# kongan/PL-SLAM-plucker

Measured on AMD Instinct MI355X. Metric: LM iterations/sec (and ms/iter) on local-BA window; final χ² vs g2o, higher is better.
Workload: dtype f64; 1 GPU; C3: 100 KF (10 fixed) / 20000 points / 4000 Plücker lines, 93975+18441 edges; one independent window per GPU; edges=112416, survey_nominal_edges=120000, trials_per_lba=23, factorisation=two-sided column-lane band LDLT (bw 7), parallelism=1 independent windows (1 per GPU)

## Files before the change

### pl-slam-plucker_amd/csrc/plba.hip

```cpp
#include <hip/hip_runtime.h>
#include <rccl/rccl.h>

#include <algorithm>
#include <chrono>
#include <cmath>
#include <cstdarg>
#include <cstdio>
#include <cstring>
#include <limits>
#include <map>
#include <mutex>
#include <numeric>
#include <string>
#include <type_traits>
#include <utility>
#include <vector>

#include "../../include/plba.h"
#include "plba_build.hpp"
#include "plba_kernels.hpp"
#include "plba_plan.hpp"
#include "plba_scratch.hpp"

namespace plba {
// ... 944 lines not shown
        d.bcr_sl[1] = N * (int64_t)bcr_xrec(bw);
        d.bcr_sl[2] = N * (int64_t)bcr_X_doubles(bw);
        d.bcr_sl[3] = 2 * N;
        d.bcr_sl[4] = kBcrCtl;
        d.bcr_sl[5] = N * (int64_t)kBcrStamps;
        ALLOC(d.bcr_pub, (size_t)W * d.bcr_sl[0]);
        ALLOC(d.bcr_x, (size_t)W * d.bcr_sl[1]);
        ALLOC(d.bcr_X, (size_t)W * d.bcr_sl[2]);
        h.h_kf.assign(nf, 0);
        for (int k = 0; k < n_kf; ++k)
            if (ws.kf_hidx[k] >= 0) h.h_kf[ws.kf_hidx[k]] = k;
        UPLOAD(d.h_kf, h.h_kf);
        ZALLOC(d.bcr_flag, (size_t)W * d.bcr_sl[3]);
        ZALLOC(d.bcr_ctl, (size_t)W * kBcrCtl);
        ZALLOC(d.bcr_stamps, (size_t)W * d.bcr_sl[5]);
        ALLOC(ctx->bk_T, (size_t)n_kf * 12);
        ALLOC(ctx->bk_X, (size_t)std::max(n_lm, 1) * 4);
        ALLOC(ctx->bk_xp, (size_t)std::max(n, 6));
        ALLOC(ctx->bk_xk, (size_t)n_kf * 6);
        ALLOC(ctx->bk_Lpb, (size_t)std::max(n_ln, 1) * 8);
        ALLOC(ctx->bk_XL, (size_t)std::max(n_ln_g, 1) * 6);
        ALLOC(ctx->bk_level, (size_t)std::max(E, 1));
        ALLOC(ctx->bk_xl, (size_t)std::max(n_lm, 1) * 4);
    }
    if (!d.band_mode) ZALLOC(d.bcr_stamps, kBcrStamps);
    ALLOC(d.bs, (size_t)W * n);
    for (int b = 0; b < nbx; ++b) ZALLOC(d.xpb[b], std::max(n, 6));
    ALLOC(d.Wbuf, (size_t)std::max(n, 1) * (kTile + 1));
    UPLOAD(d.tile_first, bp.tile_first);
    UPLOAD(d.tile_last, bp.tile_last);
    ALLOC(d.part_chi2, d.n_lin_blocks);
    ALLOC(d.part_any, d.n_lm_blocks);
    ALLOC(d.part_max, nf + d.n_lm_blocks);
    ALLOC(d.pose_part, (size_t)std::max(nf, 1) * kPoseParts * kPP);
    ALLOC(d.part_lm, (size_t)W * sl_lms(d));
    ALLOC(d.part_lms, (size_t)W * sl_lms(d));
    const int nred = kPoseParts * nf + (d.n_lm > 0 ? d.n_lm_blocks : 0), ngrp = (nred + kRedGrp - 1) / kRedGrp;
    ZALLOC(d.cnt, 2 + (size_t)nblk + nf + ngrp);
    ZALLOC(d.cnt_rcs, (size_t)W * nblk);
    ALLOC(d.wg_red, 3 * (size_t)std::max(nred, 1));
    ALLOC(d.grp_red, 3 * (size_t)std::max(ngrp, 1));
    d.n_ps = std::max(d.n_kf_blocks, d.bcr_N);
    ZALLOC(d.part_ps, (size_t)W * d.n_ps);
    ZALLOC(d.ctrl, 1);
    ALLOC(d.trace, kTraceCap);
    ALLOC(ctx->d_depth, Ep);
    ALLOC(d.red_rcs, (size_t)nblk * 36 + (size_t)nf * 6);
    ALLOC(d.red_dec, 3);
    if (d.sharded) {
        ALLOC(d.red_rcs_loc, (size_t)nblk * 36 + (size_t)nf * 6);
        ALLOC(d.red_dec_loc, 4);
    }
    d.xg_P = 0;
    if (d.sharded && xg.rng.size()) {
        d.xg_P = xg.P;
        UPLOAD(d.xg_rng, xg.rng);
        ZALLOC(d.xg_send, (size_t)(d.xg_host ? R : 1) * xg.P);
        ALLOC(d.xg_recv, (size_t)R * xg.P);
    }
    UPLOAD_D(d.lm_gpos, ctx->lm_gpos, wb.lm_gpos, n_lm);
    UPLOAD_D(d.e_gpos, ws.e_gpos, wb.e_gpos, E);
    if (d.sharded) {
        ALLOC(d.gat, (size_t)d.n_lm_g * 4 + 3 * (size_t)d.E_g);
    } else {
        ALLOC(ctx->d_outd, out_doubles(n_kf, n_pt, n_ln, E) + ((size_t)Ep + E + 7) / 8);
    }
#if defined(PLBA_STAMPS) || defined(PLBA_PHASE_STAMPS) || defined(PLBA_LMS_STAMPS)
    ZALLOC(d.stamps, 17 * 8);
#endif
}
#undef ALLOC
#undef ZALLOC
#undef UPLOAD
#undef UPLOAD_D
int stage_arrays(plba_ctx *ctx, const plba_graph *g, const WindowStructure &ws, const BlockPattern &bp,
                 const ShardRanges &xg, PhaseLog &mark) {
    StagedHost h;
    stage_state_arrays(ctx, g, ws, h);
    stage_system_arrays(ctx, g, ws, bp, xg, h);
    mark("host arrays staged");
    return ctx->commit_plan();
}
void bind_views(Dev &d) {
    const size_t nf = (size_t)d.nf;
    d.xp = d.xpb[0];
    d.xl = d.xlb[0];
    d.chi2_last = d.chi2b[0];
    if (d.sharded) {
        d.Hpp = nullptr;
        d.Hdg = d.red_iter;
        d.bp = d.red_iter + nf * 6;
        d.pact = d.red_iter + nf * 12;
        d.Hdg_w = d.red_iter_loc;
        d.bp_w = d.red_iter_loc + nf * 6;
        d.pact_w = d.red_iter_loc + nf * 12;
    } else {
        d.Hpp = d.red_iter;
        d.bp = d.red_iter + nf * 36;
        d.pact = d.red_iter + nf * 42;
        d.red_iter_loc = d.red_iter;
// ... 79 lines not shown
        return PLBA_OK;
    }
    ctx->set_error("sharded window without a transport");
    return PLBA_E_COMM;
}
int allgather(plba_ctx *ctx, const double *send, double *recv, size_t P) {
    auto &c = ctx->comm;
    if (P == 0) return PLBA_OK;
    if (c.kind == plba_ctx::Comm::RCCL) {
        const ncclResult_t r = ncclAllGather(send, recv, P, ncclDouble, c.nccl, ctx->stream);
        if (r != ncclSuccess) {
            ctx->set_error("ncclAllGather(%zu doubles): %s", P, ncclGetErrorString(r));
            return PLBA_E_COMM;
        }
        return PLBA_OK;
    }
    return allreduce(ctx, send, recv, (size_t)c.nranks * P);
}
#define COMM(send, recv, n)                                                        \
    do {                                                                           \
        int _crc = 0;                                                              \
        LAUNCH(K_COMM, _crc = allreduce(ctx, (send), (recv), (size_t)(n)));        \
        if (_crc) return _crc;                                                     \
    } while (0)

bool chunk_half(const plba_ctx *ctx) { return (long long)ctx->d.nch > ctx->tuning.chunk_half_min; }
int launch_step(plba_ctx *ctx) {
    Dev &d = ctx->d;
    hipStream_t s = ctx->stream;
    const bool chunk_direct = ctx->tuning.chunk_direct;

    if (d.E > 0) LAUNCH(K_LINEARIZE, hipLaunchKernelGGL(k_linearize, dim3(d.n_lin_blocks), dim3(kBlock), 0, s, d));
    if (d.nf > 0 || d.n_lm > 0) {
        const int nred = kPoseParts * d.nf + (d.n_lm > 0 ? d.n_lm_blocks : 0);
        LAUNCH(K_REDUCE, hipLaunchKernelGGL(k_iter_reduce, dim3(nred), dim3(kLmBlock), 0, s, d));
    }
    if (d.sharded) {
        LAUNCH(K_PACK, hipLaunchKernelGGL(k_iter_pack, dim3(1), dim3(kInitNT), 0, s, d));
        COMM(d.red_iter_loc, d.red_iter, (size_t)d.nf * 13 + 2 + d.nranks);
    }
    const bool reduced = d.nf > 0 || d.n_lm > 0;
    if (!(d.fold_init && reduced))
        LAUNCH(K_ITER_INIT, hipLaunchKernelGGL(k_iter_init, dim3(1), dim3(kInitNT), 0, s, d));
    if (d.n_lm > 0) {
        LAUNCH(K_ESCHUR, hipLaunchKernelGGL(k_edge_schur, dim3(d.n_lin_blocks, d.spec_max), dim3(kBlock), 0, s, d));
    }
    if (d.n > 0) {
        if (!d.band_mode) LAUNCH(K_MEMSET, (void)hipMemsetAsync(d.Ad, 0, sizeof(double) * (size_t)d.n * d.n, s));
        if (d.nch > 0) LAUNCH(K_ASSEMBLE, hipLaunchKernelGGL(chunk_direct ? k_rcs_chunk<false> : chunk_half(ctx) ? k_rcs_chunk_h : k_rcs_chunk<true>, dim3(8 * ((d.nch + 7) / 8), d.spec_max), dim3(64), 0, s, d));
        if (d.sharded) {
            LAUNCH(K_PACK, hipLaunchKernelGGL(k_rcs_blockpart, dim3(blocks_for(d.nblk * 42)), dim3(kBlock), 0, s, d));
            if (d.xg_P > 0) {
                int grc = 0;
                LAUNCH(K_COMM, grc = allgather(ctx, d.xg_send, d.xg_recv, (size_t)d.xg_P));
                if (grc) return grc;
                LAUNCH(K_FINALIZE, hipLaunchKernelGGL(k_rcs_xunpack, dim3(blocks_for(d.nblk * 36 + d.nf * 6)), dim3(kBlock), 0, s, d));
            } else {
                COMM(d.red_rcs_loc, d.red_rcs, (size_t)d.nblk * 36 + (size_t)d.nf * 6);
            }
        }
        if (!(d.fold && d.nch > 0))
            LAUNCH(K_FINALIZE, hipLaunchKernelGGL(k_rcs_finalize, dim3(blocks_for(d.nblk * 42)), dim3(kBlock), 0, s, d));
        const size_t solve_lds = d.n <= d.solve_lds_n ? sizeof(double) * (size_t)d.n : 0;
        if (d.band_mode) {
            hipError_t fe = hipSuccess;
            LAUNCH(K_FACTOR, fe = launch_band(d, s));
            if (fe != hipSuccess) {
                (void)hipGetLastError();
// ... 779 lines not shown
        PLBA_CHECK(d2h(ctx, res->kf_x, d.xk[ctx->cur], sizeof(double) * (size_t)d.n_kf * 6));
    }
    if (gba && res->ln_line3d && ctx->n_ln)
        PLBA_CHECK(d2h(ctx, res->ln_line3d, d.XL[ctx->cur], sizeof(double) * (size_t)ctx->n_ln * 6));
    return plba_download(ctx, res->kf_Tcw, res->pt_xyz, gba ? nullptr : res->ln_orth);
}

int plba_get_trace(plba_ctx *ctx, plba_iter_trace *out, int32_t cap, int32_t *n) {
    if (!ctx) return PLBA_E_INVALID;
    if (n) *n = (int32_t)ctx->trace.size();
    if (out)
        for (int i = 0; i < (int)ctx->trace.size() && i < cap; ++i) out[i] = ctx->trace[i];
    return PLBA_OK;
}

int plba_synchronize(plba_ctx *ctx) {
    if (!ctx) return PLBA_E_INVALID;
    PLBA_CHECK(hipStreamSynchronize(ctx->stream));
    return PLBA_OK;
}

int plba_kernel_times(plba_ctx *ctx, const char **names, double *ms, int32_t *launches, int32_t cap, int32_t *n) {
    if (!ctx) return PLBA_E_INVALID;
    if (n) *n = K_COUNT;
    for (int k = 0; k < K_COUNT && k < cap; ++k) {
        if (names) names[k] = kKernelNames[k];
        if (ms) ms[k] = ctx->k_ms[k];
        if (launches) launches[k] = ctx->k_n[k];
    }
    return PLBA_OK;
}

int plba_debug_stamps(plba_ctx *ctx, unsigned long long *out ) {
#if defined(PLBA_STAMPS) || defined(PLBA_PHASE_STAMPS) || defined(PLBA_LMS_STAMPS)
    if (!ctx || !ctx->d.stamps) return PLBA_E_STATE;
    PLBA_CHECK(d2h(ctx, out, ctx->d.stamps, 17 * 8 * sizeof(unsigned long long)));
    return PLBA_OK;
#else
    (void)ctx; (void)out;
    return PLBA_E_STATE;
#endif
}

int plba_debug_bcr_stamps(plba_ctx *ctx, unsigned long long *out, int32_t cap, int32_t *rows) {
    if (!ctx || !out || !rows) return PLBA_E_INVALID;
    if (!ctx->uploaded || !ctx->d.bcr_stamps) return PLBA_E_STATE;
    const int rows_ = std::max(ctx->d.bcr_N, 1);
    const int n = std::min(cap / kBcrStamps, rows_);
    *rows = rows_;
    PLBA_CHECK(d2h(ctx, out, ctx->d.bcr_stamps, sizeof(unsigned long long) * (size_t)n * kBcrStamps));
    return PLBA_OK;
}

int plba_structure_stats(plba_ctx *ctx, int64_t *out, int32_t cap) {
    if (!ctx || !out) return PLBA_E_INVALID;
    if (!ctx->uploaded) return PLBA_E_STATE;
    const int64_t v[22] = {ctx->d.nf, ctx->d.bw, ctx->d.nblk, (int64_t)ctx->n_triples, ctx->d.E, ctx->d.n_lm,
                           ctx->d.band_mode, ctx->d.nch, ctx->n_free_edges, ctx->d.Ep,
                           ctx->step_exec != nullptr, ctx->d.sharded, ctx->d.twisted, ctx->d.cl, ctx->d.bcr_N,
                           ctx->d.dense_mfma, ctx->bcr_fallbacks, ctx->d.spec_max, ctx->d.spec_policy,
                           ctx->h_ctrl ? ctx->h_ctrl->steps : 0, ctx->d.bcr_fused, ctx->dev_build};
    for (int i = 0; i < cap && i < 22; ++i) out[i] = v[i];
    return PLBA_OK;
}

int plba_factor_plan(int32_t bw, int32_t nf, int32_t resident, int32_t flags, int32_t *out, int32_t cap) {
    if (!out || bw < 0 || nf < 0) return PLBA_E_INVALID;
// ... 208 lines not shown
```

### pl-slam-plucker_amd/csrc/plba_dev.hpp

```cpp
#pragma once

#include <hip/hip_runtime.h>
#include <stdint.h>

#include "../../include/plba.h"
#include "plba_math.hpp"

namespace plba {

constexpr int kBlock = 256;
constexpr int kLmBlock = 64;
constexpr int kChunk = 256;
constexpr int kTraceCap = 64;
constexpr int kTile = 32;
constexpr int kBandMax = 27;
constexpr int kBandNT = 768;
__host__ __device__ constexpr int band_nt(int bw) { return bw <= 24 ? kBandNT : 512; }
__host__ __device__ constexpr int band_ur(int bw) { return band_nt(bw) <= 512 ? 6 : 3; }
constexpr int kMaxSpec = 4;
constexpr int kNB = kMaxSpec + 1;

enum LmKind : int32_t {
    kLmG2o = 0,
    kLmLbaPlucker = 1,
// ... 75 lines not shown
    int32_t bw, band_mode;
    int32_t dense_mfma;
    int32_t ring;
    unsigned long long *stamps;
    int32_t *first_blk;
    double *Bd;
    double *Lband;
    double *Kinv;
    double *zb;
    double *part_chi2;
    double *wg_red, *grp_red;
    int32_t *part_any;
    double *part_max;
    double *part_lm, *part_lms;
    double *part_ps;
    int32_t n_ps;
    int32_t fold;
    int32_t fold_init;
    int32_t *cnt;
    int32_t *h_kf;
    Ctrl *ctrl;
    plba_iter_trace *trace;
    int32_t sharded, nranks, rank;
    int32_t n_lm_g, E_g;
    double *red_iter, *red_iter_loc;
    double *red_rcs, *red_rcs_loc;
    double *xg_send, *xg_recv;
    int64_t *xg_rng;
    int64_t xg_P;
    int32_t xg_host;
    double *red_dec, *red_dec_loc;
    double *Hpp_w, *bp_w;
    double *Hdg, *Hdg_w;
    double *pose_part;
    double *pact, *pact_w;
    int32_t *lm_gpos, *e_gpos;
    double *gat;
    int32_t cl;
    int32_t diag;
    int32_t twisted, tw_m;
    double *Bd2, *bs2;
    double *Lband2, *Kinv2, *zb2;
    double *tw_sep;
    int32_t *tw_fail, *tw_count;
    int32_t bcr, bcr_N;
    int32_t bcr_fused;
    double *bcr_pub;
    double *bcr_x;
    double *bcr_X;
    uint32_t *bcr_flag;
    uint32_t *bcr_ctl;
    unsigned long long *bcr_stamps;
    int64_t bcr_sl[6];
};


__device__ __forceinline__ double *Tcur(const Dev &d) { return d.Tb[d.ctrl->cur]; }
__device__ __forceinline__ double *Xcur(const Dev &d) { return d.Xb[d.ctrl->cur]; }
__device__ __forceinline__ double *chi2cur(const Dev &d) { return d.chi2b[d.ctrl->chi_src]; }

__host__ __device__ __forceinline__ size_t sl_band(const Dev &d) { return d.band_mode ? (size_t)d.nf * (d.bw + 1) * 36 : 1; }
__host__ __device__ __forceinline__ size_t sl_tw(const Dev &d) { return (size_t)d.nf * (d.bw + 1) * 36; }
__host__ __device__ __forceinline__ size_t sl_sep(const Dev &d) {
    return 2 * ((size_t)d.bw * (d.bw + 1) * 36 + (size_t)d.bw * 6);
}
__host__ __device__ __forceinline__ size_t sl_chp(const Dev &d) { return (size_t)(d.nch > 1 ? d.nch : 1) * 42; }
__host__ __device__ __forceinline__ size_t sl_lms(const Dev &d) { return (size_t)(d.n_lms_blocks > 1 ? d.n_lms_blocks : 1); }
// ... 156 lines not shown
```

### pl-slam-plucker_amd/csrc/plba_kernels.hpp

```cpp
#pragma once

#include "plba_dev.hpp"

namespace plba {

__global__ __launch_bounds__(kBlock) void k_linearize(Dev d) {
    ITER_GUARD
    __shared__ double sh[kBlock / 64];
    const int e = blockIdx.x * kBlock + threadIdx.x;
    double rc = 0.0;
    const Ctrl *cc = d.ctrl;
    const bool sw = cc->switch_pending;
    const int nxt = cc->stage + 1;
    const int robust = sw ? cc->stage_robust[nxt] : cc->robust;
    double *chi2e = chi2cur(d);
    __shared__ __attribute__((aligned(16))) double stA[kBlock * 12], stc[kBlock * 2], stB[kBlock * 8];
    if (e < d.E) {
        double *A = stA + threadIdx.x * 12, *c = stc + threadIdx.x * 2, *B = stB + threadIdx.x * 8;
        if (sw) {
            const double stale = chi2e[e];
            for (int b = 0; b < d.nbx; ++b)
                if (d.chi2b[b] != chi2e) d.chi2b[b][e] = stale;
            if (cc->stage_classify[nxt]) {
                bool bad = stale > kChi2Thr;
// ... 80 lines not shown
            const double s = sqrt(rho1 * info);
            const bool pose_free = d.e_hidx[e] >= 0;
#pragma unroll
            for (int k = 0; k < 12; ++k) A[k] = pose_free ? s * Jp[k] : 0.0;
            c[0] = -s * err[0];
            c[1] = -s * err[1];
#pragma unroll
            for (int k = 0; k < 8; ++k) B[k] = s * Jl[k];
        } else {
#pragma unroll
            for (int k = 0; k < 12; ++k) A[k] = 0.0;
            c[0] = c[1] = 0.0;
#pragma unroll
            for (int k = 0; k < 8; ++k) B[k] = 0.0;
        }
    }
    __syncthreads();
    {
        const int e0 = blockIdx.x * kBlock, n = min(kBlock, d.E - e0);
        auto copy_out = [&](const double *src, double *dst, int cnt) {
            const double2 *s2 = reinterpret_cast<const double2 *>(src);
            double2 *d2 = reinterpret_cast<double2 *>(dst);
            for (int t = threadIdx.x; t < cnt / 2; t += kBlock) d2[t] = s2[t];
        };
        copy_out(stA, d.A + (size_t)e0 * 12, n * 12);
        copy_out(stc, d.cvec + (size_t)e0 * 2, n * 2);
        copy_out(stB, d.B + (size_t)e0 * 8, n * 8);
    }
    double s = block_sum<kBlock>(rc, sh);
    if (threadIdx.x == 0) d.part_chi2[blockIdx.x] = s;
}

constexpr int kPoseParts = 4;
constexpr int kPoseKU = 4;
constexpr int kPP = 28;
constexpr int kInitNT = 1024;

__device__ __forceinline__ constexpr int pk(int r, int c) { return r * (r + 1) / 2 + c; }

__device__ __forceinline__ double pose_partial(const Dev &d, int h, int part) {
    double acc[kPP];
#pragma unroll
    for (int k = 0; k < kPP; ++k) acc[k] = 0.0;
    constexpr int S = kPoseParts * 64, kU = kPoseKU;
    const int pend = d.pe_off[h + 1];
    for (int p0 = d.pe_off[h] + part * 64 + threadIdx.x; p0 < pend; p0 += kU * S) {
        int ei[kU];
#pragma unroll
        for (int j = 0; j < kU; ++j) ei[j] = p0 + j * S < pend ? d.pe_list[p0 + j * S] : -1;
        double a[kU][12], cv[kU][2];
#pragma unroll
        for (int j = 0; j < kU; ++j) {
            const int e = ei[j] < 0 ? ei[0] : ei[j];
            const double *A = d.A + (size_t)e * 12;
#pragma unroll
            for (int k = 0; k < 12; ++k) a[j][k] = A[k];
            cv[j][0] = d.cvec[(size_t)e * 2];
            cv[j][1] = d.cvec[(size_t)e * 2 + 1];
        }
#pragma unroll
        for (int j = 0; j < kU; ++j) {
            if (ei[j] < 0) break;
            acc[27] += d.e_active[ei[j]] ? 1.0 : 0.0;
            const double *a0 = a[j], *a1 = a[j] + 6;
            int idx = 0;
#pragma unroll
            for (int r = 0; r < 6; ++r)
#pragma unroll
                for (int cc = r; cc < 6; ++cc) acc[idx++] += a0[r] * a0[cc] + a1[r] * a1[cc];
#pragma unroll
            for (int r = 0; r < 6; ++r) acc[21 + r] += a0[r] * cv[j][0] + a1[r] * cv[j][1];
        }
    }
    {
        const int lane = threadIdx.x;
        double v[32];
#pragma unroll
        for (int k = 0; k < 32; ++k) v[k] = k < kPP ? acc[k] : 0.0;
#pragma unroll
        for (int n = 16; n >= 1; n >>= 1) {
            const int m = 2 * n;
            const bool hi = (lane & m) != 0;
#pragma unroll
            for (int i = 0; i < n; ++i) {
                const double keep = hi ? v[n + i] : v[i], send = hi ? v[i] : v[n + i];
                v[i] = keep + __shfl_xor(send, m, 64);
            }
        }
        v[0] += __shfl_xor(v[0], 1, 64);
        if ((lane & 1) == 0 && lane / 2 < kPP)
            st_sc1(d.pose_part + ((size_t)h * kPoseParts + part) * kPP + lane / 2, v[0]);
    }
    if ((d.fold_init || d.sharded) && arrive_last(d.cnt + 2 + d.nblk + h, kPoseParts)) {
        const int k = threadIdx.x;
        double v = 0.0;
        if (k < kPP) {
            const double *src = d.pose_part + (size_t)h * kPoseParts * kPP + k;
            double p[kPoseParts];
#pragma unroll
            for (int j = 0; j < kPoseParts; ++j) p[j] = ld_sc1(src + j * kPP);
            v = p[0];
#pragma unroll
            for (int j = 1; j < kPoseParts; ++j) v += p[j];
            if (k < 21) {
                int r = 0, rem = k;
                while (rem >= 6 - r) { rem -= 6 - r; ++r; }
                const int cc = r + rem;
                d.Hpp_w[(size_t)h * 36 + r * 6 + cc] = v;
                d.Hpp_w[(size_t)h * 36 + cc * 6 + r] = v;
                if (r == cc && d.Hdg_w) d.Hdg_w[(size_t)h * 6 + r] = v;
                if (r != cc) v = 0.0;
            } else if (k < 27) {
                d.bp_w[(size_t)h * 6 + (k - 21)] = v;
                v = 0.0;
            } else {
                d.pact_w[h] = v;
                v = 0.0;
            }
        }
        const double m = wave_max(fabs(v));
        if (threadIdx.x == 0) st_sc1(d.part_max + h, m);
        return m;
    }
    return 0.0;
}

__device__ __forceinline__ void landmark_reduce(const Dev &d, int lb, double &mx_out, int &any_out) {
    __shared__ double sh[kLmBlock / 64];
    const int l = lb * kLmBlock + threadIdx.x;
    const bool sw = d.ctrl->switch_pending;
    double mx = 0.0;
    bool any = false;
    if (l < d.n_lm) {
        if (sw) {
            bool act = false;
            for (int e = d.lm_off[l]; e < d.lm_off[l + 1]; ++e) act = act || d.e_active[e];
            d.lm_active[l] = act ? 1 : 0;
        }
        any = d.lm_active[l] != 0;
        if (l >= d.n_pt && lm_endpoint_lines(d.ctrl->hlm)) {
            double H6[21], b6[6];
#pragma unroll
            for (int k = 0; k < 21; ++k) H6[k] = 0.0;
#pragma unroll
            for (int k = 0; k < 6; ++k) b6[k] = 0.0;
            for (int e = d.lm_off[l]; e < d.lm_off[l + 1]; ++e) {
                double bb[6];
#pragma unroll
                for (int k = 0; k < 6; ++k) bb[k] = d.B[(size_t)e * 8 + k];
                const double c0 = d.cvec[(size_t)e * 2];
#pragma unroll
                for (int r = 0; r < 6; ++r) {
#pragma unroll
                    for (int cc = 0; cc <= r; ++cc) H6[pk(r, cc)] += bb[r] * bb[cc];
                    b6[r] += bb[r] * c0;
                }
            }
            const int li = l - d.n_pt;
#pragma unroll
            for (int k = 0; k < 21; ++k) d.Hl6[(size_t)li * 21 + k] = H6[k];
#pragma unroll
            for (int k = 0; k < 6; ++k) d.bl6[(size_t)li * 6 + k] = b6[k];
// ... 5 lines not shown
        for (int k = 0; k < 10; ++k) H[k] = 0.0;
#pragma unroll
        for (int k = 0; k < 4; ++k) b[k] = 0.0;
        const int e1 = d.lm_off[l + 1];
        for (int e0 = d.lm_off[l]; e0 < e1; e0 += 2) {
            double bb[2][8], cc2[2][2];
#pragma unroll
            for (int j = 0; j < 2; ++j) {
                const int e = e0 + j < e1 ? e0 + j : e0;
#pragma unroll
                for (int k = 0; k < 8; ++k) bb[j][k] = d.B[(size_t)e * 8 + k];
                cc2[j][0] = d.cvec[(size_t)e * 2];
                cc2[j][1] = d.cvec[(size_t)e * 2 + 1];
            }
#pragma unroll
            for (int j = 0; j < 2; ++j) {
                if (e0 + j >= e1) break;
                const double *b0 = bb[j], *b1 = bb[j] + 4;
#pragma unroll
                for (int r = 0; r < 4; ++r) {
#pragma unroll
                    for (int cc = 0; cc <= r; ++cc) H[pk(r, cc)] += b0[r] * b0[cc] + b1[r] * b1[cc];
                    b[r] += b0[r] * cc2[j][0] + b1[r] * cc2[j][1];
                }
            }
        }
#pragma unroll
        for (int k = 0; k < 10; ++k) d.Hll[(size_t)l * 10 + k] = H[k];
#pragma unroll
        for (int k = 0; k < 4; ++k) d.bl[(size_t)l * 4 + k] = b[k];
        mx = fmax(fmax(fabs(H[pk(0, 0)]), fabs(H[pk(1, 1)])), fmax(fabs(H[pk(2, 2)]), fabs(H[pk(3, 3)])));
        }
    }
    double m = block_max<kLmBlock>(mx, sh);
    const int anyb = __syncthreads_or(any ? 1 : 0);
    if (threadIdx.x == 0) {
        st_sc1(d.part_max + d.nf + lb, m);
        __hip_atomic_store(d.part_any + lb, anyb, __ATOMIC_RELAXED, __HIP_MEMORY_SCOPE_AGENT);
    }
    mx_out = m;
    any_out = anyb;
}


template <int NT, bool SC1 = false>
__device__ __forceinline__ double pose_combine(const Dev &d, double *H, double *bp) {
    double m = 0.0;
    for (int i = threadIdx.x; i < d.nf * kPP; i += NT) {
        const int h = i / kPP, k = i % kPP;
        const double *src = d.pose_part + (size_t)h * kPoseParts * kPP + k;
        double v = SC1 ? ld_sc1(src) : src[0];
#pragma unroll
        for (int j = 1; j < kPoseParts; ++j) v += SC1 ? ld_sc1(src + j * kPP) : src[j * kPP];
        if (k < 21) {
            int r = 0, rem = k;
            while (rem >= 6 - r) { rem -= 6 - r; ++r; }
            const int cc = r + rem;
            H[(size_t)h * 36 + r * 6 + cc] = v;
            H[(size_t)h * 36 + cc * 6 + r] = v;
            if (r == cc) m = fmax(m, fabs(v));
        } else if (k < 27) {
            bp[(size_t)h * 6 + (k - 21)] = v;
        } else {
            d.pact_w[h] = v;
        }
    }
    return m;
}

__global__ __launch_bounds__(kInitNT) void k_iter_pack(Dev d) {
    ITER_GUARD
    __shared__ double sh[kInitNT / 64];
    double s = 0.0;
    for (int i = threadIdx.x; i < d.n_lin_blocks; i += kInitNT) s += d.part_chi2[i];
    const double chi = block_sum<kInitNT>(s, sh);
    double m = 0.0;
    for (int i = threadIdx.x; i < d.n_lm_blocks; i += kInitNT) m = fmax(m, d.part_max[d.nf + i]);
    const double mx = block_max<kInitNT>(m, sh);
    int any = 0;
    for (int i = threadIdx.x; i < d.n_lm_blocks; i += kInitNT) any |= d.part_any[i];
    any = __syncthreads_or(any);
    double *o = d.red_iter_loc + (size_t)d.nf * 13;
    if (threadIdx.x == 0) {
        o[0] = chi;
        o[1] = any ? 1.0 : 0.0;
    }
    for (int r = threadIdx.x; r < d.nranks; r += kInitNT) o[2 + r] = r == d.rank ? mx : 0.0;
}

__device__ __forceinline__ void iter_init_ctrl(const Dev &d, double chi, double mx, bool any);
template <int NT>
__device__ __forceinline__ void iter_init_body(const Dev &d, double *sh) {
    double chi, mx;
    bool any;
    if (d.sharded) {
        const double *o = d.red_iter + (size_t)d.nf * 13;
        double m = 0.0;
        for (int i = threadIdx.x; i < d.nf * 6; i += NT) m = fmax(m, fabs(d.Hdg[i]));
        for (int r = threadIdx.x; r < d.nranks; r += NT) m = fmax(m, o[2 + r]);
        mx = block_max<NT>(m, sh);
        chi = o[0];
        any = o[1] != 0.0;
    } else {
        double m = pose_combine<NT>(d, d.Hpp_w, d.bp_w);
        double s = 0.0;
        for (int i = threadIdx.x; i < d.n_lin_blocks; i += NT) s += d.part_chi2[i];
        chi = block_sum<NT>(s, sh);
        for (int i = threadIdx.x; i < d.n_lm_blocks; i += NT) m = fmax(m, d.part_max[d.nf + i]);
        mx = block_max<NT>(m, sh);
        int a = 0;
        for (int i = threadIdx.x; i < d.n_lm_blocks; i += NT) a |= d.part_any[i];
        any = __syncthreads_or(a) != 0;
    }
    if (threadIdx.x == 0) iter_init_ctrl(d, chi, mx, any);
}
__device__ __forceinline__ void iter_init_ctrl(const Dev &d, double chi, double mx, bool any) {
    {
        Ctrl *c = d.ctrl;
        if (c->switch_pending) {
            c->switch_pending = 0;
            c->stage += 1;
            c->iter = 0;
            c->robust = c->stage_robust[c->stage];
            c->level = c->stage_level[c->stage];
            if (!any) {
                c->iters_done[c->stage] = -1;
                c->chi2_final[c->stage] = 0.0;
                c->need_iter = 0;
                if (c->stage + 1 < c->n_stages) c->switch_pending = 1;
                else c->all_done = 1;
                return;
            }
        }
        if (lm_hand_rolled(c->hlm)) {
            const double err = chi / (c->hlm == kLmLbaEndpoints && c->iter > 0 ? c->hlm_nobs2 : c->hlm_nobs);
            c->hlm_lin += 1;
            if (c->iter == 0) {
                c->maxdiag = mx;
                c->lambda = c->hlm_lambda0 * (c->hlm == kLmGba ? (double)(long long)mx : mx);
            } else if (fabs(err - c->err_prev) < c->hlm_minchg || err < c->hlm_minerr) {
                if (c->ntrace < kTraceCap)
// ... 2 lines not shown
                c->chi2_final[c->stage] = err;
                c->need_iter = 0;
                c->all_done = 1;
                return;
            }
            c->currentChi = err;
            c->chi2_start = err;
            c->lambda_start = c->lambda;
            c->accept = 0;
            c->need_iter = 0;
            return;
        }
        if (c->iter == 0) {
            c->currentChi = chi;
            c->maxdiag = mx;
            c->lambda = d.tau * mx;
            c->ni = 2.0;
        }
        c->chi2_start = c->currentChi;
        c->lambda_start = c->lambda;
        c->qmax = 0;
        c->accept = 0;
        c->rho = 0.0;
        c->broke = 0;
        c->need_iter = 0;
    }
}
__global__ __launch_bounds__(kInitNT) void k_iter_init(Dev d) {
    ITER_GUARD
    __shared__ double sh[kInitNT / 64];
    iter_init_body<kInitNT>(d, sh);
}

constexpr int kRedGrp = 256;
__device__ __forceinline__ bool iter_init_fast(const Dev &d) {
    const Ctrl *c = d.ctrl;
    return d.fold_init && !d.sharded && !lm_hand_rolled(c->hlm) && !c->switch_pending && c->iter > 0;
}
__global__ __launch_bounds__(kLmBlock) void k_iter_reduce(Dev d) {
    ITER_GUARD
    __shared__ double sh_init[kLmBlock / 64];
    const int b = blockIdx.x, np = kPoseParts * d.nf;
    const int G = (int)gridDim.x, lane = threadIdx.x;
    double sc = 0.0;
    if (d.fold_init && !iter_init_fast(d)) {
        const int lo = (int)((long long)b * d.n_lin_blocks / G), hi = (int)((long long)(b + 1) * d.n_lin_blocks / G);
        for (int i = lo + lane; i < hi; i += kLmBlock) sc += d.part_chi2[i];
    }
    double wmax = 0.0;
    int wany = 0;
    if (b < np) wmax = pose_partial(d, b / kPoseParts, b % kPoseParts);
    else landmark_reduce(d, b - np, wmax, wany);
    if (!d.fold_init) return;
    if (iter_init_fast(d)) return;
    {
        sc = wave_sum(sc);
        if (lane == 0) {
            st_sc1(d.wg_red + 3 * (size_t)b, sc);
            st_sc1(d.wg_red + 3 * (size_t)b + 1, wmax);
            st_sc1(d.wg_red + 3 * (size_t)b + 2, wany ? 1.0 : 0.0);
        }
    }
    constexpr int U = kRedGrp / kLmBlock;
    const int g = b / kRedGrp, gn = min(kRedGrp, G - kRedGrp * g), ng = (G + kRedGrp - 1) / kRedGrp;
    if (!arrive_last(d.cnt + 2 + d.nblk + d.nf + g, gn)) return;
    {
        double cv[U], mv[U], av[U];
#pragma unroll
        for (int u = 0; u < U; ++u) {
            const int k = lane * U + u;
            const double *w = d.wg_red + 3 * (size_t)(kRedGrp * g + min(k, gn - 1));
            cv[u] = ld_sc1(w);
            mv[u] = ld_sc1(w + 1);
            av[u] = ld_sc1(w + 2);
        }
        double c = 0.0, m = 0.0, a = 0.0;
#pragma unroll
        for (int u = 0; u < U; ++u)
            if (lane * U + u < gn) {
                c += cv[u];
                m = fmax(m, mv[u]);
                a = fmax(a, av[u]);
            }
        c = wave_sum(c);
        m = wave_max(m);
        a = wave_max(a);
        if (lane == 0) {
            st_sc1(d.grp_red + 3 * (size_t)g, c);
            st_sc1(d.grp_red + 3 * (size_t)g + 1, m);
            st_sc1(d.grp_red + 3 * (size_t)g + 2, a);
        }
    }
    if (!arrive_last(d.cnt + 1, ng)) return;
    double c = 0.0, m = 0.0, a = 0.0;
    for (int g0 = 0; g0 < ng; g0 += 64) {
        double cg = 0.0, mg = 0.0, ag = 0.0;
        if (g0 + lane < ng) {
            const double *w = d.grp_red + 3 * (size_t)(g0 + lane);
            cg = ld_sc1(w);
            mg = ld_sc1(w + 1);
            ag = ld_sc1(w + 2);
        }
        c += wave_sum(cg);
        m = fmax(m, wave_max(mg));
        a = fmax(a, wave_max(ag));
    }
    (void)sh_init;
    if (lane == 0) iter_init_ctrl(d, c, m, a != 0.0);
}

}

#include "plba_rcs.hpp"
#include "plba_dense.hpp"
#include "plba_band.hpp"
#include "plba_band_cl.hpp"
#include "plba_bcr.hpp"
#include "plba_pgo.hpp"

namespace plba {

__global__ __launch_bounds__(kBlock) void k_pose_update(Dev d0) {
    TRIAL_SLOT(0)
    if (blockIdx.x == 0) pose_update_wg<kBlock>(d, false);
}

__device__ __forceinline__ void lm_chol(const Dev &d, int l, double lam, bool mul, double (&L)[10], double (&g)[4],
                                        double (&S)[4], bool sgn = false) {
    const int DIM = is_point_lm(d, l) ? 3 : 4;
    double H[10];
#pragma unroll
    for (int k = 0; k < 10; ++k) { H[k] = d.Hll[(size_t)l * 10 + k]; L[k] = 0.0; }
#pragma unroll
    for (int k = 0; k < 4; ++k) { g[k] = 0.0; S[k] = 1.0; }
#pragma unroll
    for (int j = 0; j < 4; ++j) {
        if (j < DIM) {
            double sj = H[pk(j, j)] + (mul ? lam * H[pk(j, j)] : lam);
#pragma unroll
            for (int p = 0; p < j; ++p) sj -= (L[pk(j, p)] * S[p]) * L[pk(j, p)];
// ... 796 lines not shown
```

### pl-slam-plucker_amd/plba/roofline.py

```python
from __future__ import annotations

from .synth import Graph

F = 8
I = 4


def state_bytes(g: Graph) -> int:
    return g.n_kf * 12 * F + g.n_pt * 3 * F + g.n_ln * 4 * F


def kernel_bytes(g: Graph, name: str, st: dict) -> float:
    E, Ep, El = g.n_ept + g.n_eln, g.n_ept, g.n_eln
    Ef = st.get("free_edges", E)
    n_lm = g.n_pt + g.n_ln
    nf = st.get("nf", int((g.kf_fixed == 0).sum()))
    bw = st.get("bw", 7)
    T = st.get("triples", 0)
    nblk = st.get("nblk", 0)
    nch = st.get("chunks", 0)
    blk = 36 * F
    if name == "k_linearize":
        rd = Ep * (2 * I + 2 * F + F + 1 + I) + El * (2 * I + 4 * F + F + 1 + I) + state_bytes(g)
        return rd + E * (12 + 2 + 8 + 1) * F
    if name == "k_iter_reduce":
        return (Ef * (I + 14 * F) + nf * 4 * 27 * F
                + E * (8 + 2) * F + n_lm * (I + (10 + 4) * F))
    if name == "k_iter_init":
        return nf * 4 * 27 * F + nf * (36 + 6) * F
    if name == "k_edge_schur":
        return E * (I + 8 * F + 10 * F) + n_lm * (10 + 4) * F
    if name == "k_rcs_chunk":
        return E * (12 + 8 + 2) * F + T * 2 * I + nch * 42 * F
    if name == "k_rcs_finalize":
        return nch * 42 * F + nf * (36 + 6) * F + nblk * blk + nf * 6 * F
    if name in ("k_rcs_factor", "k_rcs_factor_band", "k_rcs_factor_twisted"):
        return (nf * (bw + 1) * blk + nf * 6 * F + nf * bw * blk + nf * (36 + 6 + 6) * F
                + g.n_kf * (12 + 12) * F + nf * 6 * F)
    if name == "k_rcs_factor_bcr":
        S = 6 * bw
        N = -(-nf // max(bw, 1))
        NG = (2 * bw + 1) * (2 * bw + 2) // 2 - 1
        return (nf * (bw + 1) * blk + nf * 6 * F + (N - 1) * 36 * NG * F * 3 + N * S * F * 3
                + nf * 6 * F + g.n_kf * (12 + 12) * F + nf * 6 * F)
    if name == "k_pose_update":
        return g.n_kf * (12 + 12) * F + nf * 12 * F
    if name == "k_lm_solve":
        ev = Ep * (I + 1 + 2 * F + F) + El * (I + 1 + 4 * F + F) + E * F + g.n_kf * 12 * F
        return n_lm * (4 + 4 + 10 + 4 + 4) * F + n_lm * I + Ef * (I + (12 + 8) * F) + nf * 6 * F + ev
    return 0.0
```

Baseline: 5478 LM iterations/s.

## Fuse per-pose partial reductions into one workgroup via LDS instead of global atomics

k_iter_reduce now runs one 256-thread workgroup per free pose, with four waves, in place of four separate 64-thread workgroups. The four pose partials are combined in shared memory behind a barrier. Before, they went through global pose_part storage plus an arrive-last atomic counter, and pose_combine ran again in iter_init. Landmark blocks are packed four waves per workgroup, and the grouped final reduction uses groups of 64. The aim is to cut the workgroup count, global round-trips and atomic synchronisation in the per-iteration reduction. Optional cycle-counter instrumentation (PLBA_IRP_STAMPS) is also added.

```diff
diff --git a/pl-slam-plucker_amd/csrc/plba.hip b/pl-slam-plucker_amd/csrc/plba.hip
--- a/pl-slam-plucker_amd/csrc/plba.hip
+++ b/pl-slam-plucker_amd/csrc/plba.hip
@@ -1000,11 +1000,10 @@
     ALLOC(d.part_chi2, d.n_lin_blocks);
     ALLOC(d.part_any, d.n_lm_blocks);
     ALLOC(d.part_max, nf + d.n_lm_blocks);
-    ALLOC(d.pose_part, (size_t)std::max(nf, 1) * kPoseParts * kPP);
     ALLOC(d.part_lm, (size_t)W * sl_lms(d));
     ALLOC(d.part_lms, (size_t)W * sl_lms(d));
-    const int nred = kPoseParts * nf + (d.n_lm > 0 ? d.n_lm_blocks : 0), ngrp = (nred + kRedGrp - 1) / kRedGrp;
-    ZALLOC(d.cnt, 2 + (size_t)nblk + nf + ngrp);
+    const int nred = iter_reduce_wgs(d), ngrp = (nred + kRedGrp - 1) / kRedGrp;
+    ZALLOC(d.cnt, 2 + (size_t)ngrp);
     ZALLOC(d.cnt_rcs, (size_t)W * nblk);
     ALLOC(d.wg_red, 3 * (size_t)std::max(nred, 1));
     ALLOC(d.grp_red, 3 * (size_t)std::max(ngrp, 1));
@@ -1033,7 +1032,9 @@
     } else {
         ALLOC(ctx->d_outd, out_doubles(n_kf, n_pt, n_ln, E) + ((size_t)Ep + E + 7) / 8);
     }
-#if defined(PLBA_STAMPS) || defined(PLBA_PHASE_STAMPS) || defined(PLBA_LMS_STAMPS)
+#if defined(PLBA_IRP_STAMPS) && PLBA_IRP_STAMPS == 2
+    ZALLOC(d.stamps, 17 * 8 + (size_t)nf * (1 + kPoseParts * kPP));
+#elif defined(PLBA_STAMPS) || defined(PLBA_PHASE_STAMPS) || defined(PLBA_LMS_STAMPS) || defined(PLBA_IRP_STAMPS)
     ZALLOC(d.stamps, 17 * 8);
 #endif
 }
@@ -1179,8 +1180,7 @@
 
     if (d.E > 0) LAUNCH(K_LINEARIZE, hipLaunchKernelGGL(k_linearize, dim3(d.n_lin_blocks), dim3(kBlock), 0, s, d));
     if (d.nf > 0 || d.n_lm > 0) {
-        const int nred = kPoseParts * d.nf + (d.n_lm > 0 ? d.n_lm_blocks : 0);
-        LAUNCH(K_REDUCE, hipLaunchKernelGGL(k_iter_reduce, dim3(nred), dim3(kLmBlock), 0, s, d));
+        LAUNCH(K_REDUCE, hipLaunchKernelGGL(k_iter_reduce, dim3(iter_reduce_wgs(d)), dim3(kRedNT), 0, s, d));
     }
     if (d.sharded) {
         LAUNCH(K_PACK, hipLaunchKernelGGL(k_iter_pack, dim3(1), dim3(kInitNT), 0, s, d));
@@ -2026,7 +2026,7 @@
 }
 
 int plba_debug_stamps(plba_ctx *ctx, unsigned long long *out ) {
-#if defined(PLBA_STAMPS) || defined(PLBA_PHASE_STAMPS) || defined(PLBA_LMS_STAMPS)
+#if defined(PLBA_STAMPS) || defined(PLBA_PHASE_STAMPS) || defined(PLBA_LMS_STAMPS) || defined(PLBA_IRP_STAMPS)
     if (!ctx || !ctx->d.stamps) return PLBA_E_STATE;
     PLBA_CHECK(d2h(ctx, out, ctx->d.stamps, 17 * 8 * sizeof(unsigned long long)));
     return PLBA_OK;
diff --git a/pl-slam-plucker_amd/csrc/plba_dev.hpp b/pl-slam-plucker_amd/csrc/plba_dev.hpp
--- a/pl-slam-plucker_amd/csrc/plba_dev.hpp
+++ b/pl-slam-plucker_amd/csrc/plba_dev.hpp
@@ -131,7 +131,6 @@
     double *red_dec, *red_dec_loc;
     double *Hpp_w, *bp_w;
     double *Hdg, *Hdg_w;
-    double *pose_part;
     double *pact, *pact_w;
     int32_t *lm_gpos, *e_gpos;
     double *gat;
diff --git a/pl-slam-plucker_amd/csrc/plba_kernels.hpp b/pl-slam-plucker_amd/csrc/plba_kernels.hpp
--- a/pl-slam-plucker_amd/csrc/plba_kernels.hpp
+++ b/pl-slam-plucker_amd/csrc/plba_kernels.hpp
@@ -136,22 +136,44 @@
 }
 
 constexpr int kPoseParts = 4;
+constexpr int kRedNT = 64 * kPoseParts;
 constexpr int kPoseKU = 4;
 constexpr int kPP = 28;
 constexpr int kInitNT = 1024;
+__host__ __device__ __forceinline__ int iter_reduce_wgs(const Dev &d) {
+    return d.nf + (d.n_lm > 0 ? (d.n_lm_blocks + kPoseParts - 1) / kPoseParts : 0);
+}
 
 __device__ __forceinline__ constexpr int pk(int r, int c) { return r * (r + 1) / 2 + c; }
 
-__device__ __forceinline__ double pose_partial(const Dev &d, int h, int part) {
+#ifdef PLBA_IRP_STAMPS
+#define IRP_T(v)                                           \
+    asm volatile("s_waitcnt vmcnt(0) lgkmcnt(0)" ::: "memory"); \
+    const unsigned long long v = __builtin_readcyclecounter()
+#define IRP_ACC(acc, t1, t0) acc += (t1) - (t0)
+#else
+#define IRP_T(v)
+#define IRP_ACC(acc, t1, t0)
+#endif
+
+__device__ __forceinline__ double pose_reduce(const Dev &d, int h) {
+    __shared__ double sh_pose[kPoseParts][kPP];
+    const int part = threadIdx.x >> 6, lane = threadIdx.x & 63;
+#ifdef PLBA_IRP_STAMPS
+    unsigned long long irp_idx = 0, irp_gat = 0, irp_sum = 0;
+#endif
+    IRP_T(it0);
     double acc[kPP];
 #pragma unroll
     for (int k = 0; k < kPP; ++k) acc[k] = 0.0;
     constexpr int S = kPoseParts * 64, kU = kPoseKU;
     const int pend = d.pe_off[h + 1];
-    for (int p0 = d.pe_off[h] + part * 64 + threadIdx.x; p0 < pend; p0 += kU * S) {
+    for (int p0 = d.pe_off[h] + part * 64 + lane; p0 < pend; p0 += kU * S) {
+        IRP_T(ia);
         int ei[kU];
 #pragma unroll
         for (int j = 0; j < kU; ++j) ei[j] = p0 + j * S < pend ? d.pe_list[p0 + j * S] : -1;
+        IRP_T(ib);
         double a[kU][12], cv[kU][2];
 #pragma unroll
         for (int j = 0; j < kU; ++j) {
@@ -162,6 +184,7 @@
             cv[j][0] = d.cvec[(size_t)e * 2];
             cv[j][1] = d.cvec[(size_t)e * 2 + 1];
         }
+        IRP_T(ic);
 #pragma unroll
         for (int j = 0; j < kU; ++j) {
             if (ei[j] < 0) break;
@@ -175,9 +198,14 @@
 #pragma unroll
             for (int r = 0; r < 6; ++r) acc[21 + r] += a0[r] * cv[j][0] + a1[r] * cv[j][1];
         }
-    }
+        IRP_T(id);
+        IRP_ACC(irp_idx, ib, ia);
+        IRP_ACC(irp_gat, ic, ib);
+        IRP_ACC(irp_sum, id, ic);
+    }
+    IRP_T(it1);
+    double v0;
     {
-        const int lane = threadIdx.x;
         double v[32];
 #pragma unroll
         for (int k = 0; k < 32; ++k) v[k] = k < kPP ? acc[k] : 0.0;
@@ -191,21 +219,41 @@
                 v[i] = keep + __shfl_xor(send, m, 64);
             }
         }
-        v[0] += __shfl_xor(v[0], 1, 64);
-        if ((lane & 1) == 0 && lane / 2 < kPP)
-            st_sc1(d.pose_part + ((size_t)h * kPoseParts + part) * kPP + lane / 2, v[0]);
-    }
-    if ((d.fold_init || d.sharded) && arrive_last(d.cnt + 2 + d.nblk + h, kPoseParts)) {
-        const int k = threadIdx.x;
+        v0 = v[0] + __shfl_xor(v[0], 1, 64);
+    }
+    IRP_T(it2);
+    bool combiner = part == 0;
+#if defined(PLBA_IRP_STAMPS) && PLBA_IRP_STAMPS == 2
+    {
+        __shared__ int sh_last[kPoseParts];
+        int32_t *counter = reinterpret_cast<int32_t *>(d.stamps + 17 * 8 + h);
+        double *pp = reinterpret_cast<double *>(d.stamps + 17 * 8 + d.nf) + (size_t)h * kPoseParts * kPP;
+        if ((lane & 1) == 0 && lane / 2 < kPP) st_sc1(pp + part * kPP + lane / 2, v0);
+        asm volatile("s_waitcnt vmcnt(0)" ::: "memory");
+        if (lane == 0) {
+            const int32_t old = __hip_atomic_fetch_add(counter, 1, __ATOMIC_RELAXED, __HIP_MEMORY_SCOPE_AGENT);
+            sh_last[part] = old == kPoseParts - 1 ? 1 : 0;
+            if (sh_last[part]) __hip_atomic_store(counter, 0, __ATOMIC_RELAXED, __HIP_MEMORY_SCOPE_AGENT);
+        }
+        wave_lds_sync();
+        combiner = sh_last[part] != 0;
+        if (combiner && lane < kPP)
+            for (int j = 0; j < kPoseParts; ++j) sh_pose[j][lane] = ld_sc1(pp + j * kPP + lane);
+        wave_lds_sync();
+    }
+#else
+    if ((lane & 1) == 0 && lane / 2 < kPP) sh_pose[part][lane / 2] = v0;
+    lds_barrier();
+#endif
+    IRP_T(it3);
+    double m = 0.0;
+    if (combiner) {
+        const int k = lane;
         double v = 0.0;
         if (k < kPP) {
-            const double *src = d.pose_part + (size_t)h * kPoseParts * kPP + k;
-            double p[kPoseParts];
-#pragma unroll
-            for (int j = 0; j < kPoseParts; ++j) p[j] = ld_sc1(src + j * kPP);
-            v = p[0];
-#pragma unroll
-            for (int j = 1; j < kPoseParts; ++j) v += p[j];
+            v = sh_pose[0][k];
+#pragma unroll
+            for (int j = 1; j < kPoseParts; ++j) v += sh_pose[j][k];
             if (k < 21) {
                 int r = 0, rem = k;
                 while (rem >= 6 - r) { rem -= 6 - r; ++r; }
@@ -222,16 +270,28 @@
                 v = 0.0;
             }
         }
-        const double m = wave_max(fabs(v));
-        if (threadIdx.x == 0) st_sc1(d.part_max + h, m);
-        return m;
-    }
-    return 0.0;
-}
-
-__device__ __forceinline__ void landmark_reduce(const Dev &d, int lb, double &mx_out, int &any_out) {
-    __shared__ double sh[kLmBlock / 64];
-    const int l = lb * kLmBlock + threadIdx.x;
+        m = wave_max(fabs(v));
+        if (lane == 0) d.part_max[h] = m;
+    }
+#ifdef PLBA_IRP_STAMPS
+    IRP_T(it4);
+    if (lane == 0 && d.stamps) {
+        unsigned long long *st = d.stamps + 14 * 8;
+        atomicAdd(st + 0, irp_idx);
+        atomicAdd(st + 1, irp_gat);
+        atomicAdd(st + 2, irp_sum + (it2 - it1));
+        atomicAdd(st + 3, it3 - it2);
+        if (combiner) atomicAdd(st + 4, it4 - it3);
+        atomicAdd(st + 5, 1ull);
+        atomicAdd(st + 6, it4 - it0);
+        if (combiner) atomicAdd(st + 7, 1ull);
+    }
+#endif
+    return m;
+}
+
+__device__ __forceinline__ void landmark_reduce(const Dev &d, int lg, double &mx_out, int &any_out) {
+    const int l = lg * kLmBlock + (threadIdx.x & 63);
     const bool sw = d.ctrl->switch_pending;
     double mx = 0.0;
     bool any = false;
@@ -303,41 +363,16 @@
         mx = fmax(fmax(fabs(H[pk(0, 0)]), fabs(H[pk(1, 1)])), fmax(fabs(H[pk(2, 2)]), fabs(H[pk(3, 3)])));
         }
     }
-    double m = block_max<kLmBlock>(mx, sh);
-    const int anyb = __syncthreads_or(any ? 1 : 0);
-    if (threadIdx.x == 0) {
-        st_sc1(d.part_max + d.nf + lb, m);
-        __hip_atomic_store(d.part_any + lb, anyb, __ATOMIC_RELAXED, __HIP_MEMORY_SCOPE_AGENT);
+    const double m = wave_max(mx);
+    const int anyb = __ballot(any) != 0 ? 1 : 0;
+    if ((threadIdx.x & 63) == 0 && lg < d.n_lm_blocks) {
+        d.part_max[d.nf + lg] = m;
+        d.part_any[lg] = anyb;
     }
     mx_out = m;
     any_out = anyb;
 }
 
-
-template <int NT, bool SC1 = false>
-__device__ __forceinline__ double pose_combine(const Dev &d, double *H, double *bp) {
-    double m = 0.0;
-    for (int i = threadIdx.x; i < d.nf * kPP; i += NT) {
-        const int h = i / kPP, k = i % kPP;
-        const double *src = d.pose_part + (size_t)h * kPoseParts * kPP + k;
-        double v = SC1 ? ld_sc1(src) : src[0];
-#pragma unroll
-        for (int j = 1; j < kPoseParts; ++j) v += SC1 ? ld_sc1(src + j * kPP) : src[j * kPP];
-        if (k < 21) {
-            int r = 0, rem = k;
-            while (rem >= 6 - r) { rem -= 6 - r; ++r; }
-            const int cc = r + rem;
-            H[(size_t)h * 36 + r * 6 + cc] = v;
-            H[(size_t)h * 36 + cc * 6 + r] = v;
-            if (r == cc) m = fmax(m, fabs(v));
-        } else if (k < 27) {
-            bp[(size_t)h * 6 + (k - 21)] = v;
-        } else {
-            d.pact_w[h] = v;
-        }
-    }
-    return m;
-}
 
 __global__ __launch_bounds__(kInitNT) void k_iter_pack(Dev d) {
     ITER_GUARD
@@ -373,11 +408,11 @@
         chi = o[0];
         any = o[1] != 0.0;
     } else {
-        double m = pose_combine<NT>(d, d.Hpp_w, d.bp_w);
         double s = 0.0;
         for (int i = threadIdx.x; i < d.n_lin_blocks; i += NT) s += d.part_chi2[i];
         chi = block_sum<NT>(s, sh);
-        for (int i = threadIdx.x; i < d.n_lm_blocks; i += NT) m = fmax(m, d.part_max[d.nf + i]);
+        double m = 0.0;
+        for (int i = threadIdx.x; i < d.nf + d.n_lm_blocks; i += NT) m = fmax(m, d.part_max[i]);
         mx = block_max<NT>(m, sh);
         int a = 0;
         for (int i = threadIdx.x; i < d.n_lm_blocks; i += NT) a |= d.part_any[i];
@@ -446,59 +481,54 @@
     iter_init_body<kInitNT>(d, sh);
 }
 
-constexpr int kRedGrp = 256;
+constexpr int kRedGrp = 64;
 __device__ __forceinline__ bool iter_init_fast(const Dev &d) {
     const Ctrl *c = d.ctrl;
     return d.fold_init && !d.sharded && !lm_hand_rolled(c->hlm) && !c->switch_pending && c->iter > 0;
 }
-__global__ __launch_bounds__(kLmBlock) void k_iter_reduce(Dev d) {
+__global__ __launch_bounds__(kRedNT) void k_iter_reduce(Dev d) {
     ITER_GUARD
-    __shared__ double sh_init[kLmBlock / 64];
-    const int b = blockIdx.x, np = kPoseParts * d.nf;
-    const int G = (int)gridDim.x, lane = threadIdx.x;
+    __shared__ double sh_red[kPoseParts][3];
+    const int b = blockIdx.x, G = (int)gridDim.x;
+    const int wave = threadIdx.x >> 6, lane = threadIdx.x & 63;
+    const int GW = kPoseParts * d.nf + (d.n_lm > 0 ? d.n_lm_blocks : 0), bw = kPoseParts * b + wave;
     double sc = 0.0;
-    if (d.fold_init && !iter_init_fast(d)) {
-        const int lo = (int)((long long)b * d.n_lin_blocks / G), hi = (int)((long long)(b + 1) * d.n_lin_blocks / G);
-        for (int i = lo + lane; i < hi; i += kLmBlock) sc += d.part_chi2[i];
+    if (d.fold_init && !iter_init_fast(d) && bw < GW) {
+        const int lo = (int)((long long)bw * d.n_lin_blocks / GW), hi = (int)((long long)(bw + 1) * d.n_lin_blocks / GW);
+        for (int i = lo + lane; i < hi; i += 64) sc += d.part_chi2[i];
     }
     double wmax = 0.0;
     int wany = 0;
-    if (b < np) wmax = pose_partial(d, b / kPoseParts, b % kPoseParts);
-    else landmark_reduce(d, b - np, wmax, wany);
+    if (b < d.nf) wmax = pose_reduce(d, b);
+    else landmark_reduce(d, kPoseParts * (b - d.nf) + wave, wmax, wany);
     if (!d.fold_init) return;
     if (iter_init_fast(d)) return;
-    {
-        sc = wave_sum(sc);
-        if (lane == 0) {
-            st_sc1(d.wg_red + 3 * (size_t)b, sc);
-            st_sc1(d.wg_red + 3 * (size_t)b + 1, wmax);
-            st_sc1(d.wg_red + 3 * (size_t)b + 2, wany ? 1.0 : 0.0);
-        }
-    }
-    constexpr int U = kRedGrp / kLmBlock;
+    sc = wave_sum(sc);
+    if (lane == 0) {
+        sh_red[wave][0] = sc;
+        sh_red[wave][1] = wmax;
+        sh_red[wave][2] = wany ? 1.0 : 0.0;
+    }
+    lds_barrier();
+    if (threadIdx.x == 0) {
+        double c = 0.0, m = 0.0, a = 0.0;
+#pragma unroll
+        for (int w = 0; w < kPoseParts; ++w) {
+            c += sh_red[w][0];
+            m = fmax(m, sh_red[w][1]);
+            a = fmax(a, sh_red[w][2]);
+        }
+        st_sc1(d.wg_red + 3 * (size_t)b, c);
+        st_sc1(d.wg_red + 3 * (size_t)b + 1, m);
+        st_sc1(d.wg_red + 3 * (size_t)b + 2, a);
+    }
     const int g = b / kRedGrp, gn = min(kRedGrp, G - kRedGrp * g), ng = (G + kRedGrp - 1) / kRedGrp;
-    if (!arrive_last(d.cnt + 2 + d.nblk + d.nf + g, gn)) return;
-    {
-        double cv[U], mv[U], av[U];
-#pragma unroll
-        for (int u = 0; u < U; ++u) {
-            const int k = lane * U + u;
-            const double *w = d.wg_red + 3 * (size_t)(kRedGrp * g + min(k, gn - 1));
-            cv[u] = ld_sc1(w);
-            mv[u] = ld_sc1(w + 1);
-            av[u] = ld_sc1(w + 2);
-        }
-        double c = 0.0, m = 0.0, a = 0.0;
-#pragma unroll
-        for (int u = 0; u < U; ++u)
-            if (lane * U + u < gn) {
-                c += cv[u];
-                m = fmax(m, mv[u]);
-                a = fmax(a, av[u]);
-            }
-        c = wave_sum(c);
-        m = wave_max(m);
-        a = wave_max(a);
+    if (!arrive_last(d.cnt + 2 + g, gn)) return;
+    if (wave == 0) {
+        const double *w = d.wg_red + 3 * (size_t)(kRedGrp * g + min(lane, gn - 1));
+        const double cv = ld_sc1(w), mv = ld_sc1(w + 1), av = ld_sc1(w + 2);
+        const bool in = lane < gn;
+        const double c = wave_sum(in ? cv : 0.0), m = wave_max(in ? mv : 0.0), a = wave_max(in ? av : 0.0);
         if (lane == 0) {
             st_sc1(d.grp_red + 3 * (size_t)g, c);
             st_sc1(d.grp_red + 3 * (size_t)g + 1, m);
@@ -506,6 +536,7 @@
         }
     }
     if (!arrive_last(d.cnt + 1, ng)) return;
+    if (wave != 0) return;
     double c = 0.0, m = 0.0, a = 0.0;
     for (int g0 = 0; g0 < ng; g0 += 64) {
         double cg = 0.0, mg = 0.0, ag = 0.0;
@@ -519,7 +550,6 @@
         m = fmax(m, wave_max(mg));
         a = fmax(a, wave_max(ag));
     }
-    (void)sh_init;
     if (lane == 0) iter_init_ctrl(d, c, m, a != 0.0);
 }
 
diff --git a/pl-slam-plucker_amd/plba/roofline.py b/pl-slam-plucker_amd/plba/roofline.py
--- a/pl-slam-plucker_amd/plba/roofline.py
+++ b/pl-slam-plucker_amd/plba/roofline.py
@@ -24,10 +24,10 @@
         rd = Ep * (2 * I + 2 * F + F + 1 + I) + El * (2 * I + 4 * F + F + 1 + I) + state_bytes(g)
         return rd + E * (12 + 2 + 8 + 1) * F
     if name == "k_iter_reduce":
-        return (Ef * (I + 14 * F) + nf * 4 * 27 * F
+        return (Ef * (I + 14 * F) + nf * (36 + 6 + 2) * F
                 + E * (8 + 2) * F + n_lm * (I + (10 + 4) * F))
     if name == "k_iter_init":
-        return nf * 4 * 27 * F + nf * (36 + 6) * F
+        return (nf + (n_lm + 63) // 64 + (E + 255) // 256) * F
     if name == "k_edge_schur":
         return E * (I + 8 * F + 10 * F) + n_lm * (10 + 4) * F
     if name == "k_rcs_chunk":
```

After: 5486 LM iterations/s (median of 6 runs). No clear change (+0.1%).
